# TDLdefA-QUN/Noise-Resilience-in-Discrete-Time-Crystal-Realizations-on-Quantum-Computers

Measured on AMD Instinct MI355X. Metric: Floquet-periods×instances/sec at L=20; RZZ-kernel HBM GB/s vs peak, higher is better.
Workload: dtype f64

## Files before the change

noise-resilience-in-discrete-time-crystal-realizations-on-quantum-computers_amd/csrc/dtc_wavefront.hip:

```cpp
#include <hip/hip_runtime.h>

#include "dtc_device.h"
#include "dtc_kernels.h"
#include "dtc_wf_frame.h"

#ifndef DTC_WF_SPLIT
#define DTC_WF_SPLIT 1
#endif
#ifndef DTC_WF_WAVE_XCH
#define DTC_WF_WAVE_XCH 0
#endif

namespace dtc {

template <int LAY>
__device__ __forceinline__ void wf_diag(double2 (&v)[kRegs], const double2* tab, int t,
                                        double2 fac) {
  static_assert(LAY >= 0 && LAY <= 2, "tile layout");
  if (LAY == 1) {
    const int y = ybase<1>(t);
    const double2 c = cmul(fac, tab[kWfL1Reg + wf_l1_thr_index(y)]);
    const double2* tr = tab + wf_l1_reg_index(y);
#pragma unroll
    for (int r = 0; r < kRegs; ++r) v[r] = cmul(v[r], cmul(c, tr[r << 1]));
  } else if (LAY == 2) {
    const double2 c = cmul(fac, tab[t & (kWfTabA - 1)]);
    const double2* tb = tab + kWfTabA + ((t >> 6) & 3);
#pragma unroll
    for (int r = 0; r < kRegs; ++r) v[r] = cmul(v[r], cmul(c, tb[r << 2]));
  } else {
    const double2 c = cmul(fac, tab[kWfTabA + ((t >> 2) & 63)]);
    const double2* ta = tab + ((t & 7) << 4);
#pragma unroll
    for (int r = 0; r < kRegs; ++r) v[r] = cmul(v[r], cmul(c, ta[r]));
  }
}

template <int KIND>
__device__ __forceinline__ void wf_kick_lane3(double2 (&v)[kRegs], double f) {
  const long long sm = (KIND == kKindRY && (__lane_id() & 8)) ? (long long)(1ull << 63) : 0ll;
#pragma unroll
  for (int r = 0; r < kRegs; ++r) {
    const double px = xor_lane<8>(v[r].x), py = xor_lane<8>(v[r].y);
    if (KIND == kKindRX) {
      v[r] = make_double2(fma(f, v[r].x, -py), fma(f, v[r].y, px));
    } else {
      v[r] = make_double2(fma(f, v[r].x, __longlong_as_double(__double_as_longlong(px) ^ sm)),
                          fma(f, v[r].y, __longlong_as_double(__double_as_longlong(py) ^ sm)));
    }
  }
}

template <int KIND, int QM0, bool SPLIT>
__global__ __launch_bounds__(kThreads, SPLIT ? 3 : 2) void dtc_wf_pass(WfArgs A) {
  __shared__ double2 s_tile[SPLIT ? 1 : kTile];
  __shared__ double s_half[SPLIT ? kHalfSlots : 1];
  __shared__ double2 s_tab[(kWfSteps + 1) * kWfTab];

  const int t = threadIdx.x;
  const int og = A.octet_bits;
  const int64_t b = og ? (((int64_t)blockIdx.y << 3) | (blockIdx.x & 7)) : (int64_t)blockIdx.y;
  const int64_t tile = og ? (int64_t)(blockIdx.x >> 3) : (int64_t)blockIdx.x;
  if (b >= A.batch) return;
  const int inst = (int)((A.batch_start + b) / A.n_traj);
  const int n = A.n_steps;
  constexpr bool kTwoLay = kWfT2Lay1 && QM0 == 8;

  TileMap M;
  M.c = A.c;
  M.s = A.s;
  M.cmask = (1 << A.c) - 1;
  const int mid = A.s - A.c;
  M.tbase = ((tile & (((int64_t)1 << mid) - 1)) << A.c) | ((tile >> mid) << (A.s + kTileBits - A.c));

  const int var = A.out_bit >= 0 ? (int)((M.tbase >> A.out_bit) & 1) : 0;
  const double2* tg = A.tab + ((int64_t)inst * (kWfSteps + 1) * 2 + var) * kWfTab;
  double2 stage[kWfSteps + 1];
#pragma unroll
  for (int st = 0; st <= kWfSteps; ++st) {
    stage[st] = make_double2(1.0, 0.0);
    if (t < kWfTab && ((A.dmask >> st) & 1)) stage[st] = tg[st * 2 * kWfTab + t];
  }

  const int64_t sbase = state_base(b, A.state_len, og);
  const int64_t vofs = octet_spread(M.at(ybase<2>(t)), og);
  double2 v[kRegs];
  {
    const double2* src = A.src + sbase + vofs;
#pragma unroll
    for (int r = 0; r < kRegs; ++r) {
      const d2v w =
          __builtin_nontemporal_load((const d2v*)(src + octet_spread(M.rel(r << 8), og)));
      v[r] = make_double2(w.x, w.y);
    }
  }
  const RecScalar R0(A.recs + b * kRecPerState);
  const RecScalar R1(A.recs + ((int64_t)A.batch + b) * kRecPerState);
  const long long fxd = R1.bits(8 * kRecTotal + kWfMaskXD);
  const int fzx = R1.i(kRecTotal, kWfMaskZX);
  if (t < kWfTab) {
    const int last = 31 - __builtin_clz(A.dmask | 1);
    const int fz = fzx & (kTile - 1);
    const bool hi = t >= kWfTabA;
    const int ti = hi ? t - kWfTabA : t;
    const int zt = hi ? fz >> 6 : fz & 63;
#pragma unroll
    for (int st = 0; st <= kWfSteps; ++st) {
      const int fx = (int)(fxd >> (kTileBits * st)) & (kTile - 1);
      if (kTwoLay && (st & 1)) {
        const bool th = t >= kWfL1Reg;
        if (t < kWfL1Reg + kWfL1Thr) {
          const int j = (th ? t - kWfL1Reg : t) ^ (th ? wf_l1_thr_index(fx) : wf_l1_reg_index(fx));
          const bool neg =
              st == last && (__popc(j & (th ? wf_l1_thr_zmask(fz) : wf_l1_reg_zmask(fz))) & 1);
          s_tab[st * kWfTab + (th ? kWfL1Reg : 0) + j] =
              neg ? make_double2(-stage[st].x, -stage[st].y) : stage[st];
        }
        continue;
      }
      const int j = ti ^ (hi ? fx >> 6 : fx & (kWfTabA - 1));
      const bool neg = st == last && (__popc(j & zt) & 1);
      s_tab[st * kWfTab + (hi ? kWfTabA : 0) + j] =
          neg ? make_double2(-stage[st].x, -stage[st].y) : stage[st];
    }
  }
  __syncthreads();

  double2 gf = cmul(make_double2(R0.d(kRecTotal, 0), R0.d(kRecTotal, 1)),
                    make_double2(R1.d(kRecTotal, 0), R1.d(kRecTotal, 1)));
  auto diag = [&](auto lay, int st) {
    if (!((A.dmask >> st) & 1)) return;
    wf_diag<decltype(lay)::value>(v, s_tab + st * kWfTab, t, gf);
    gf = make_double2(1.0, 0.0);
  };
  auto kick = [&](auto nib, int st) {
    constexpr int N = decltype(nib)::value;
    if (!(A.mask[st] & (0xFu << (4 * N)))) return;
    const RecScalar R(A.recs + ((int64_t)(st >> 1) * A.batch + b) * kRecPerState);
    apply_nibble<N, KIND, N == 0 ? QM0 : 15, true>(v, R, (st & 1) * kTileBits);
  };
  using L0 = std::integral_constant<int, 0>;
  using L1 = std::integral_constant<int, 1>;
  using L2 = std::integral_constant<int, 2>;
  constexpr bool kWaveXch = DTC_WF_WAVE_XCH != 0;

  auto kick3 = [&](int st) {
    if (!(A.mask[st] & 8u)) return;
    const RecScalar R(A.recs + ((int64_t)(st >> 1) * A.batch + b) * kRecPerState);
    wf_kick_lane3<KIND>(v, R.d((st & 1) * kTileBits + 3, 3));
  };

  if constexpr (kTwoLay) {
    bool in1 = false;
#pragma unroll 1
    for (int st = 0; st < n; st += 2) {
      diag(L2{}, st);
      kick(L2{}, st);
      xch_tile<SPLIT, 2, 1>(v, s_tile, s_half, t);
      kick(L1{}, st);
      kick3(st);
      if (st + 1 < n) {
        diag(L1{}, st + 1);
        kick3(st + 1);
        kick(L1{}, st + 1);
        xch_tile<SPLIT, 1, 2>(v, s_tile, s_half, t);
        kick(L2{}, st + 1);
      } else {
        in1 = true;
      }
    }
    if (in1) {
      diag(L1{}, n);
      xch_tile<SPLIT, 1, 2>(v, s_tile, s_half, t);
    } else {
      diag(L2{}, n);
    }
  } else {
    bool in0 = false;
#pragma unroll 1
    for (int st = 0; st < n; st += 2) {
      diag(L2{}, st);
      kick(L2{}, st);
      xch_tile<SPLIT, 2, 1>(v, s_tile, s_half, t);
      kick(L1{}, st);
      xch_tile<SPLIT, 1, 0, kWaveXch>(v, s_tile, s_half, t);
      kick(L0{}, st);
      if (st + 1 < n) {
        diag(L0{}, st + 1);
        kick(L0{}, st + 1);
        xch_tile<SPLIT, 0, 1, kWaveXch>(v, s_tile, s_half, t);
        kick(L1{}, st + 1);
        xch_tile<SPLIT, 1, 2>(v, s_tile, s_half, t);
        kick(L2{}, st + 1);
      } else {
        in0 = true;
      }
    }
    if (in0) {
      diag(L0{}, n);
      xch_tile<SPLIT, 0, 2>(v, s_tile, s_half, t);
    } else {
      diag(L2{}, n);
    }
  }
  if (!A.dmask) {
    const int fz = fzx & (kTile - 1);
    const double sg = (__popc(t & fz) & 1) ? -1.0 : 1.0;
#pragma unroll
    for (int r = 0; r < kRegs; ++r) {
      const double s = (__popc(r & (fz >> 8)) & 1) ? -sg : sg;
      v[r] = cmul(v[r], make_double2(s * gf.x, s * gf.y));
    }
  }
  {
    const int fx = (fzx >> 16) & (kTile - 1);
    const int xr = fx >> 8;
    double2* dst = A.dst + sbase + octet_spread(M.at(ybase<2>(t) ^ (fx & 255)), og);
#pragma unroll
    for (int r = 0; r < kRegs; ++r) {
      d2v x;
      x.x = v[r].x;
      x.y = v[r].y;
      __builtin_nontemporal_store(x, (d2v*)(dst + octet_spread(M.rel((r ^ xr) << 8), og)));
    }
  }
}

hipError_t launch_wavefront(const WfArgs& a, int kind, hipStream_t stream) {
  if (a.L_eff < kTileBits || a.L_eff > 32 || a.n_steps < 1 || a.n_steps > kWfSteps ||
      a.c < 0 || a.c > kTileBits || a.s < a.c || a.s + kTileBits - a.c > a.L_eff ||
      a.out_bit >= a.L_eff || a.batch < 1 || !a.tab || !a.recs || !a.src || !a.dst)
    return hipErrorInvalidValue;
  if (a.octet_bits && (a.octet_bits < 4 || a.octet_bits > a.L_eff)) return hipErrorInvalidValue;
  const bool cols3 = a.c == 3;
  if (!cols3 && a.c != kTileBits) return hipErrorInvalidValue;
  for (int st = 0; st < a.n_steps; ++st)
    if (a.mask[st] >> kTileBits || (cols3 && (a.mask[st] & 7u))) return hipErrorInvalidValue;
  if (a.dmask < 0 || a.dmask >> (a.n_steps + 1)) return hipErrorInvalidValue;
  const int n_tiles = 1 << (a.L_eff - kTileBits);
  const dim3 grid = a.octet_bits ? dim3(n_tiles * 8, (a.batch + 7) / 8) : dim3(n_tiles, a.batch);
  const dim3 block(kThreads);
  constexpr bool kSplit = DTC_WF_SPLIT != 0;
  if (kind == kKindRX) {
    if (cols3) hipLaunchKernelGGL((dtc_wf_pass<kKindRX, 8, kSplit>), grid, block, 0, stream, a);
    else hipLaunchKernelGGL((dtc_wf_pass<kKindRX, 15, kSplit>), grid, block, 0, stream, a);
  } else if (kind == kKindRY) {
    if (cols3) hipLaunchKernelGGL((dtc_wf_pass<kKindRY, 8, kSplit>), grid, block, 0, stream, a);
    else hipLaunchKernelGGL((dtc_wf_pass<kKindRY, 15, kSplit>), grid, block, 0, stream, a);
  } else {
    return hipErrorInvalidValue;
  }
  return hipGetLastError();
}

}
```

noise-resilience-in-discrete-time-crystal-realizations-on-quantum-computers_amd/csrc/dtc_wf_frame.h:

```cpp
#pragma once
#include <stdint.h>

#ifdef __HIPCC__
#define DTC_WF_HD __host__ __device__
#else
#define DTC_WF_HD
#endif

namespace dtc {

static constexpr int kWfFrameSteps = 4;
static constexpr int kWfFrameBits = 12;

struct WfFrame {
  double coef[kWfFrameSteps][kWfFrameBits];
  uint64_t xdiag;
  int zlast;
  int xend;
  int ph;
};

DTC_WF_HD inline int wf_step_bits(uint32_t mask, int act) {
  int m = 0;
  for (int n = 0; n < 3; ++n)
    if (mask & (0xFu << (4 * n))) m |= 0xF << (4 * n);
  return m & act;
}

DTC_WF_HD inline void wf_frame_walk(bool rx, int n_steps, const uint32_t* mask, int dmask,
                                    int act, const int (*var)[kWfFrameBits],
                                    const double (*coef)[kWfFrameBits], WfFrame& o) {
  auto form_a = [&](int st, int k) { return (var[st][k] >> 1) ^ 1; };
  auto zbit = [&](int st, int k) {
    return rx ? (var[st][k] & 1) : ((var[st][k] & 1) ^ form_a(st, k));
  };
  int last = n_steps;
  for (int st = 0; st < n_steps; ++st)
    if ((dmask >> st) & 1) last = st;
  if ((dmask >> n_steps) & 1) last = n_steps;
  int npost = 0;
  for (int st = last; st < n_steps; ++st) {
    const int bits = wf_step_bits(mask[st], act);
    for (int k = 0; k < kWfFrameBits; ++k)
      if ((bits >> k) & 1) npost ^= zbit(st, k) << k;
  }
  int x = 0, z = 0, ph = 0;
  o.xdiag = 0;
  o.zlast = 0;
  for (int st = 0; st <= n_steps; ++st) {
    if ((dmask >> st) & 1) o.xdiag |= (uint64_t)x << (kWfFrameBits * st);
    if (st == last) {
      o.zlast = z ^ npost;
      z = npost;
    }
    for (int k = 0; k < kWfFrameBits; ++k) {
      if (st < kWfFrameSteps) o.coef[st][k] = 0.0;
      if (st == n_steps || !((wf_step_bits(mask[st], act) >> k) & 1)) continue;
      const int fa = form_a(st, k), n2 = zbit(st, k);
      const double g = fa ? -coef[st][k] : coef[st][k];
      const int flip = ((rx ? z : (x ^ z)) >> k) & 1;
      o.coef[st][k] = flip ? -g : g;
      ph += (rx ? 3 * fa : 2 * fa) + 2 * flip;
      x ^= fa << k;
      ph += 2 * (n2 & (x >> k) & 1);
      z ^= n2 << k;
    }
  }
  for (int st = n_steps + 1; st < kWfFrameSteps; ++st)
    for (int k = 0; k < kWfFrameBits; ++k) o.coef[st][k] = 0.0;
  o.xend = x;
  o.ph = ph & 3;
}

static constexpr int kWfL1Reg = 64;
static constexpr int kWfL1Thr = 32;

DTC_WF_HD inline bool wf_l1_reg_bit(int k) { return k >= 4 && k <= 7; }
DTC_WF_HD inline int wf_l1_reg_pos(int k) { return (k >= 3 && k <= 8) ? k - 3 : -1; }
DTC_WF_HD inline int wf_l1_thr_pos(int k) { return k == 3 ? 0 : ((k >= 8 && k <= 11) ? k - 7 : -1); }
DTC_WF_HD inline int wf_l1_reg_index(int y) { return (y >> 3) & 63; }
DTC_WF_HD inline int wf_l1_thr_index(int y) { return ((y >> 3) & 1) | (((y >> 8) & 15) << 1); }
DTC_WF_HD inline int wf_l1_reg_zmask(int z) { return (z >> 3) & 63; }
DTC_WF_HD inline int wf_l1_thr_zmask(int z) { return ((z >> 9) & 7) << 2; }
DTC_WF_HD inline bool wf_l1_in_reg(int k, int k2) {
  return wf_l1_reg_bit(k) || (k2 >= 0 && wf_l1_reg_bit(k2));
}

}
#undef DTC_WF_HD
```

Before: 291,600.

## Fetch per-thread diagonal factor from global and shrink LDS table for four workgroups

The per-thread part of each diagonal phase table is no longer staged in shared memory. Each thread fetches its own factor from global memory one step ahead, and only the register-indexed part stays in LDS. This smaller LDS footprint lets the split-exchange kernel declare four workgroups per CU instead of three. The two step loops are merged into one do-while that prefetches the next diagonal factor, and sched barriers are added inside the diagonal multiply. The gain in occupancy is paid for with extra global loads per step and more register pressure, and the negation and index logic is rewritten, which risks correctness.

```diff
diff --git a/noise-resilience-in-discrete-time-crystal-realizations-on-quantum-computers_amd/csrc/dtc_wavefront.hip b/noise-resilience-in-discrete-time-crystal-realizations-on-quantum-computers_amd/csrc/dtc_wavefront.hip
--- a/noise-resilience-in-discrete-time-crystal-realizations-on-quantum-computers_amd/csrc/dtc_wavefront.hip
+++ b/noise-resilience-in-discrete-time-crystal-realizations-on-quantum-computers_amd/csrc/dtc_wavefront.hip
@@ -10,29 +10,26 @@
 #ifndef DTC_WF_WAVE_XCH
 #define DTC_WF_WAVE_XCH 0
 #endif
+#ifndef DTC_WF_WG4
+#define DTC_WF_WG4 1
+#endif
 
 namespace dtc {
 
 template <int LAY>
-__device__ __forceinline__ void wf_diag(double2 (&v)[kRegs], const double2* tab, int t,
-                                        double2 fac) {
+__device__ __forceinline__ void wf_diag(double2 (&v)[kRegs], const double2* slot, int t,
+                                        double2 fac, double2 e) {
   static_assert(LAY >= 0 && LAY <= 2, "tile layout");
-  if (LAY == 1) {
-    const int y = ybase<1>(t);
-    const double2 c = cmul(fac, tab[kWfL1Reg + wf_l1_thr_index(y)]);
-    const double2* tr = tab + wf_l1_reg_index(y);
-#pragma unroll
-    for (int r = 0; r < kRegs; ++r) v[r] = cmul(v[r], cmul(c, tr[r << 1]));
-  } else if (LAY == 2) {
-    const double2 c = cmul(fac, tab[t & (kWfTabA - 1)]);
-    const double2* tb = tab + kWfTabA + ((t >> 6) & 3);
-#pragma unroll
-    for (int r = 0; r < kRegs; ++r) v[r] = cmul(v[r], cmul(c, tb[r << 2]));
-  } else {
-    const double2 c = cmul(fac, tab[kWfTabA + ((t >> 2) & 63)]);
-    const double2* ta = tab + ((t & 7) << 4);
-#pragma unroll
-    for (int r = 0; r < kRegs; ++r) v[r] = cmul(v[r], cmul(c, ta[r]));
+  const double2 c = cmul(fac, e);
+  const double2* tr = slot + (LAY == 1   ? wf_l1_reg_index(ybase<1>(t))
+                              : LAY == 2 ? ((t >> 6) & 3)
+                                         : ((t & 7) << 4));
+  constexpr int kStep = LAY == 1 ? 2 : (LAY == 2 ? 4 : 1);
+#pragma unroll
+  for (int g = 0; g < kRegs; g += 4) {
+#pragma unroll
+    for (int r = g; r < g + 4; ++r) v[r] = cmul(v[r], cmul(c, tr[r * kStep]));
+    __builtin_amdgcn_sched_barrier(0);
   }
 }
 
@@ -51,11 +48,28 @@
   }
 }
 
+__host__ __device__ constexpr int wf_slot_ofs(bool two_lay, int st) {
+  return two_lay ? st * kWfTabB : (st >> 1) * kWfTab + (st & 1) * kWfTabB;
+}
+__host__ __device__ constexpr int wf_tab_lds(bool two_lay) { return wf_slot_ofs(two_lay, kWfSteps + 1); }
+static_assert(kWfTabB == 64 && kWfL1Reg == 64 && kWfTabA == kWfFetchTabA && (kWfSteps & 1) == 0,
+              "the register tables of dtc_wf_frame.h");
+
+__host__ __device__ constexpr bool wf_wg4(int qm0) {
+  return ((DTC_WF_WG4 >> (qm0 == 8)) & 1) &&
+         sizeof(double) * kHalfSlots + sizeof(double2) * wf_tab_lds(kWfT2Lay1 && qm0 == 8) <=
+             160 * 1024 / 4;
+}
+
 template <int KIND, int QM0, bool SPLIT>
-__global__ __launch_bounds__(kThreads, SPLIT ? 3 : 2) void dtc_wf_pass(WfArgs A) {
+__global__ __launch_bounds__(kThreads, SPLIT ? (wf_wg4(QM0) ? 4 : 3) : 2) void dtc_wf_pass(WfArgs A) {
+  constexpr bool kWg4 = SPLIT && wf_wg4(QM0);
+  constexpr bool kTwoLay = kWfT2Lay1 && QM0 == 8;
   __shared__ double2 s_tile[SPLIT ? 1 : kTile];
   __shared__ double s_half[SPLIT ? kHalfSlots : 1];
-  __shared__ double2 s_tab[(kWfSteps + 1) * kWfTab];
+  __shared__ double2 s_tab[kWg4 || !SPLIT ? wf_tab_lds(kTwoLay) : (kWfSteps + 1) * kWfTab];
+  static_assert(!kWg4 || sizeof(s_half) + sizeof(s_tab) <= 160 * 1024 / 4, "four workgroups per CU");
+  static_assert(wf_tab_lds(kTwoLay) <= (kWfSteps + 1) * kWfTab, "the padded form holds the tables");
 
   const int t = threadIdx.x;
   const int og = A.octet_bits;
@@ -64,7 +78,7 @@
   if (b >= A.batch) return;
   const int inst = (int)((A.batch_start + b) / A.n_traj);
   const int n = A.n_steps;
-  constexpr bool kTwoLay = kWfT2Lay1 && QM0 == 8;
+  constexpr int kOddLay = kTwoLay ? 1 : 0;
 
   TileMap M;
   M.c = A.c;
@@ -78,8 +92,10 @@
   double2 stage[kWfSteps + 1];
 #pragma unroll
   for (int st = 0; st <= kWfSteps; ++st) {
+    const int lay = (st & 1) ? kOddLay : 2;
     stage[st] = make_double2(1.0, 0.0);
-    if (t < kWfTab && ((A.dmask >> st) & 1)) stage[st] = tg[st * 2 * kWfTab + t];
+    if (t < wf_reg_size(lay) && ((A.dmask >> st) & 1))
+      stage[st] = tg[st * 2 * kWfTab + wf_reg_base(lay) + t];
   }
 
   const int64_t sbase = state_base(b, A.state_len, og);
@@ -98,29 +114,33 @@
   const RecScalar R1(A.recs + ((int64_t)A.batch + b) * kRecPerState);
   const long long fxd = R1.bits(8 * kRecTotal + kWfMaskXD);
   const int fzx = R1.i(kRecTotal, kWfMaskZX);
-  if (t < kWfTab) {
-    const int last = 31 - __builtin_clz(A.dmask | 1);
+  const int last = 31 - __builtin_clz(A.dmask | 1);
+  auto wf_fetch = [&](auto lay, int st) {
+    constexpr int LAY = decltype(lay)::value;
+    double2 e = make_double2(1.0, 0.0);
+    if ((A.dmask >> st) & 1) {
+      const int fx = (int)(fxd >> (kTileBits * st)) & (kTile - 1);
+      e = tg[st * 2 * kWfTab + wf_thr_fetch(LAY, ybase<LAY>(t), fx)];
+      if (st == last && wf_thr_neg(LAY, ybase<LAY>(t), fzx & (kTile - 1)))
+        e = make_double2(-e.x, -e.y);
+    }
+    return e;
+  };
+  using L0 = std::integral_constant<int, 0>;
+  using L1 = std::integral_constant<int, 1>;
+  using L2 = std::integral_constant<int, 2>;
+  using LOdd = std::integral_constant<int, kOddLay>;
+  double2 cn = wf_fetch(L2{}, 0);
+  if (t < kWfTabA) {
     const int fz = fzx & (kTile - 1);
-    const bool hi = t >= kWfTabA;
-    const int ti = hi ? t - kWfTabA : t;
-    const int zt = hi ? fz >> 6 : fz & 63;
 #pragma unroll
     for (int st = 0; st <= kWfSteps; ++st) {
+      const int lay = (st & 1) ? kOddLay : 2;
+      if (t >= wf_reg_size(lay) || !((A.dmask >> st) & 1)) continue;
       const int fx = (int)(fxd >> (kTileBits * st)) & (kTile - 1);
-      if (kTwoLay && (st & 1)) {
-        const bool th = t >= kWfL1Reg;
-        if (t < kWfL1Reg + kWfL1Thr) {
-          const int j = (th ? t - kWfL1Reg : t) ^ (th ? wf_l1_thr_index(fx) : wf_l1_reg_index(fx));
-          const bool neg =
-              st == last && (__popc(j & (th ? wf_l1_thr_zmask(fz) : wf_l1_reg_zmask(fz))) & 1);
-          s_tab[st * kWfTab + (th ? kWfL1Reg : 0) + j] =
-              neg ? make_double2(-stage[st].x, -stage[st].y) : stage[st];
-        }
-        continue;
-      }
-      const int j = ti ^ (hi ? fx >> 6 : fx & (kWfTabA - 1));
-      const bool neg = st == last && (__popc(j & zt) & 1);
-      s_tab[st * kWfTab + (hi ? kWfTabA : 0) + j] =
+      const int j = t ^ wf_reg_xmask(lay, fx);
+      const bool neg = st == last && (__popc(j & wf_reg_zmask(lay, fz)) & 1);
+      s_tab[wf_slot_ofs(kTwoLay, st) + j] =
           neg ? make_double2(-stage[st].x, -stage[st].y) : stage[st];
     }
   }
@@ -128,10 +148,12 @@
 
   double2 gf = cmul(make_double2(R0.d(kRecTotal, 0), R0.d(kRecTotal, 1)),
                     make_double2(R1.d(kRecTotal, 0), R1.d(kRecTotal, 1)));
-  auto diag = [&](auto lay, int st) {
-    if (!((A.dmask >> st) & 1)) return;
-    wf_diag<decltype(lay)::value>(v, s_tab + st * kWfTab, t, gf);
-    gf = make_double2(1.0, 0.0);
+  auto diag = [&](auto lay, int st, auto nlay, int nx) {
+    if ((A.dmask >> st) & 1) {
+      wf_diag<decltype(lay)::value>(v, s_tab + wf_slot_ofs(kTwoLay, st), t, gf, cn);
+      gf = make_double2(1.0, 0.0);
+    }
+    if (nx <= kWfSteps) cn = wf_fetch(nlay, nx);
   };
   auto kick = [&](auto nib, int st) {
     constexpr int N = decltype(nib)::value;
@@ -139,9 +161,6 @@
     const RecScalar R(A.recs + ((int64_t)(st >> 1) * A.batch + b) * kRecPerState);
     apply_nibble<N, KIND, N == 0 ? QM0 : 15, true>(v, R, (st & 1) * kTileBits);
   };
-  using L0 = std::integral_constant<int, 0>;
-  using L1 = std::integral_constant<int, 1>;
-  using L2 = std::integral_constant<int, 2>;
   constexpr bool kWaveXch = DTC_WF_WAVE_XCH != 0;
 
   auto kick3 = [&](int st) {
@@ -150,59 +169,37 @@
     wf_kick_lane3<KIND>(v, R.d((st & 1) * kTileBits + 3, 3));
   };
 
-  if constexpr (kTwoLay) {
-    bool in1 = false;
+  int st = 0;
 #pragma unroll 1
-    for (int st = 0; st < n; st += 2) {
-      diag(L2{}, st);
+  do {
+    diag(L2{}, st, LOdd{}, st + 1);
+    if (st < n) {
       kick(L2{}, st);
       xch_tile<SPLIT, 2, 1>(v, s_tile, s_half, t);
       kick(L1{}, st);
-      kick3(st);
+      if constexpr (kTwoLay) {
+        kick3(st);
+      } else {
+        xch_tile<SPLIT, 1, 0, kWaveXch>(v, s_tile, s_half, t);
+        kick(L0{}, st);
+      }
+      diag(LOdd{}, st + 1, L2{}, st + 2);
       if (st + 1 < n) {
-        diag(L1{}, st + 1);
-        kick3(st + 1);
-        kick(L1{}, st + 1);
+        if constexpr (kTwoLay) {
+          kick3(st + 1);
+          kick(L1{}, st + 1);
+        } else {
+          kick(L0{}, st + 1);
+          xch_tile<SPLIT, 0, 1, kWaveXch>(v, s_tile, s_half, t);
+          kick(L1{}, st + 1);
+        }
         xch_tile<SPLIT, 1, 2>(v, s_tile, s_half, t);
         kick(L2{}, st + 1);
-      } else {
-        in1 = true;
       }
     }
-    if (in1) {
-      diag(L1{}, n);
-      xch_tile<SPLIT, 1, 2>(v, s_tile, s_half, t);
-    } else {
-      diag(L2{}, n);
-    }
-  } else {
-    bool in0 = false;
-#pragma unroll 1
-    for (int st = 0; st < n; st += 2) {
-      diag(L2{}, st);
-      kick(L2{}, st);
-      xch_tile<SPLIT, 2, 1>(v, s_tile, s_half, t);
-      kick(L1{}, st);
-      xch_tile<SPLIT, 1, 0, kWaveXch>(v, s_tile, s_half, t);
-      kick(L0{}, st);
-      if (st + 1 < n) {
-        diag(L0{}, st + 1);
-        kick(L0{}, st + 1);
-        xch_tile<SPLIT, 0, 1, kWaveXch>(v, s_tile, s_half, t);
-        kick(L1{}, st + 1);
-        xch_tile<SPLIT, 1, 2>(v, s_tile, s_half, t);
-        kick(L2{}, st + 1);
-      } else {
-        in0 = true;
-      }
-    }
-    if (in0) {
-      diag(L0{}, n);
-      xch_tile<SPLIT, 0, 2>(v, s_tile, s_half, t);
-    } else {
-      diag(L2{}, n);
-    }
-  }
+    st += 2;
+  } while (st <= n);
+  if (n & 1) xch_tile<SPLIT, kOddLay, 2>(v, s_tile, s_half, t);
   if (!A.dmask) {
     const int fz = fzx & (kTile - 1);
     const double sg = (__popc(t & fz) & 1) ? -1.0 : 1.0;
diff --git a/noise-resilience-in-discrete-time-crystal-realizations-on-quantum-computers_amd/csrc/dtc_wf_frame.h b/noise-resilience-in-discrete-time-crystal-realizations-on-quantum-computers_amd/csrc/dtc_wf_frame.h
--- a/noise-resilience-in-discrete-time-crystal-realizations-on-quantum-computers_amd/csrc/dtc_wf_frame.h
+++ b/noise-resilience-in-discrete-time-crystal-realizations-on-quantum-computers_amd/csrc/dtc_wf_frame.h
@@ -86,5 +86,32 @@
   return wf_l1_reg_bit(k) || (k2 >= 0 && wf_l1_reg_bit(k2));
 }
 
+static constexpr int kWfFetchTabA = 128;
+DTC_WF_HD inline int wf_thr_staged(int lay, int y) {
+  return lay == 2 ? (y & (kWfFetchTabA - 1)) : (lay == 0 ? ((y >> 6) & 63) : wf_l1_thr_index(y));
+}
+DTC_WF_HD inline int wf_thr_fetch(int lay, int y, int fx) {
+  const int i = wf_thr_staged(lay, y);
+  if (lay == 2) return i ^ (fx & (kWfFetchTabA - 1));
+  if (lay == 0) return kWfFetchTabA + (i ^ ((fx >> 6) & 63));
+  return kWfL1Reg + (i ^ wf_l1_thr_index(fx));
+}
+DTC_WF_HD inline bool wf_thr_neg(int lay, int y, int fz) {
+  const int zm = lay == 2 ? (fz & 63) : (lay == 0 ? ((fz >> 6) & 63) : wf_l1_thr_zmask(fz));
+  int p = wf_thr_staged(lay, y) & zm;
+  p ^= p >> 4;
+  p ^= p >> 2;
+  p ^= p >> 1;
+  return p & 1;
+}
+DTC_WF_HD inline int wf_reg_base(int lay) { return lay == 2 ? kWfFetchTabA : 0; }
+DTC_WF_HD inline int wf_reg_size(int lay) { return lay == 0 ? kWfFetchTabA : 64; }
+DTC_WF_HD inline int wf_reg_xmask(int lay, int fx) {
+  return lay == 2 ? ((fx >> 6) & 63) : (lay == 0 ? (fx & (kWfFetchTabA - 1)) : wf_l1_reg_index(fx));
+}
+DTC_WF_HD inline int wf_reg_zmask(int lay, int fz) {
+  return lay == 2 ? ((fz >> 6) & 63) : (lay == 0 ? (fz & 63) : wf_l1_reg_zmask(fz));
+}
+
 }
 #undef DTC_WF_HD
```

Result: faster. 296,600 (median of 6 runs) (+1.7%).
